# ross39/new_bloom_filter_repo

Hardware: AMD Instinct MI355X
Metric: Mpixels/s Bloom insert+query, 1080p residuals (higher is better)
Workload: dtype u64

## Files before the change

### new_bloom_filter_repo_amd/csrc/rbf_api.hip

```cpp
#include "rbf_host.h"
#include "rbf_kernels.h"
#include "rbf_kernels_noise.h"
#include "rbf_kernels_mask.h"
#include "rbf_kernels_hold.h"
#include "rbf_kernels_lookahead.h"
#include "rbf_kernels_barrett.h"
#include "rbf_kernels_insert_f64.h"
#include "rbf_kernels_reduce.h"
#include "rbf_kernels_query_f64.h"
#include "rbf_kernels_query_f64_tiled.h"
#include "rbf_kernels_witness.h"
#include "rbf_kernels_pack.h"
#include "rbf_kernels_digest.h"
#include "rbf_kernels_cut.h"
#include "rbf_rice_host.h"

#include <cmath>

struct MaskArgs {
    const void *frames; FrameLayout l; uint32_t nframes;
    int32_t thr_floor; const int32_t *thr_floors;
    void *masks; uint64_t mask_stride; uint64_t *ones;
    uint32_t channels;
};
// ... 103 lines not shown
    HIP_TRY(hipGetLastError());
    return RBF_OK;
}

static void launch_mask_gop(rbf_ctx *ctx, const MaskArgs &a, uint64_t fast_segs, uint32_t chunks, const MaskChunks &mc,
                            const int32_t *thr_tab_fast, const MaskFinish &fin)
{
    const uint32_t bx = (uint32_t)((fast_segs + WG_WAVES - 1) / WG_WAVES), pixel = a.l.pixel_stride;
    const size_t lds = (size_t)(a.nframes - 1) * 4;
    uint64_t *const acc = ctx->ones_acc.p;
    LaunchTimer t(ctx, RBF_K_MASK);
#define RBF_MASK_GOP(S, PB, Z) hipLaunchKernelGGL((k_residual_mask_gop<S, PB, true, Z>), dim3(bx, chunks), dim3(WG_THREADS), lds, ctx->stream,   \
                               (const uint8_t *)a.frames, a.l.frame_stride, a.nframes, fast_segs, a.thr_floor, thr_tab_fast,                    \
                               (uint16_t *)a.masks, a.mask_stride / 2, acc, mc, fin)
#define RBF_MASK_GOP2(S, PB) do { if (thr0) RBF_MASK_GOP(S, PB, true); else RBF_MASK_GOP(S, PB, false); } while (0)
#define RBF_MASK_ANY_GOP(S, PB) hipLaunchKernelGGL((k_residual_mask_any_gop<S, PB, true>), dim3(bx, chunks), dim3(WG_THREADS), lds, ctx->stream, \
                                (const uint8_t *)a.frames, a.l.frame_stride, a.nframes, fast_segs, thr_tab_fast, (uint16_t *)a.masks,           \
                                a.mask_stride / 2, acc, mc, fin)
    const bool thr0 = !thr_tab_fast && a.thr_floor == 0 && !ctx->knobs.force_generic_mask_bits;
    if (a.channels >= 2) {
        if (pixel == 3) RBF_MASK_ANY_GOP(uint8_t, 3);
        else if (pixel == 4) RBF_MASK_ANY_GOP(uint8_t, 4);
        else if (pixel == 6) RBF_MASK_ANY_GOP(uint16_t, 6);
        else RBF_MASK_ANY_GOP(uint16_t, 8);
    }
    else if (a.l.sample_bytes == 1 && pixel == 1) RBF_MASK_GOP2(uint8_t, 1);
    else if (a.l.sample_bytes == 1) RBF_MASK_GOP2(uint8_t, 3);
    else if (pixel == 2) RBF_MASK_GOP2(uint16_t, 2);
    else RBF_MASK_GOP2(uint16_t, 6);
#undef RBF_MASK_ANY_GOP
#undef RBF_MASK_GOP2
#undef RBF_MASK_GOP
}

static void launch_mask_generic(rbf_ctx *ctx, const MaskArgs &a, uint64_t first_word, const int32_t *thr_tab)
{
    const uint64_t n = (uint64_t)a.l.width * a.l.height, rest = (n + 63) / 64 - first_word;
    uint64_t bx = (rest + WG_WAVES * 16 - 1) / (WG_WAVES * 16);
    if (bx < 1) bx = 1;
    if (bx > 65535) bx = 65535;
    const dim3 grid((uint32_t)bx, a.nframes - 1), block(WG_THREADS);
    LaunchTimer t(ctx, RBF_K_MASK);
    by_sample_width(a.l.sample_bytes, [&](auto s) {
        using S = decltype(s);
        if (a.channels >= 2)
            hipLaunchKernelGGL(k_residual_mask_any<S>, grid, block, 0, ctx->stream, (const uint8_t *)a.frames, a.l.frame_stride, a.l.width, n,
                               a.l.row_pitch, a.l.pixel_stride, a.channels, thr_tab, (uint64_t *)a.masks, a.mask_stride / 8, ctx->ones_acc.p, first_word);
        else
            hipLaunchKernelGGL(k_residual_mask<S>, grid, block, 0, ctx->stream, (const uint8_t *)a.frames, a.l.frame_stride, a.l.width, n,
                               a.l.row_pitch, a.l.pixel_stride, a.thr_floor, thr_tab, (uint64_t *)a.masks, a.mask_stride / 8, ctx->ones_acc.p, first_word);
    });
}

static int prepare_mask_tickets(rbf_ctx *ctx)
{
    if (ctx->mask_ticket.p) return RBF_OK;
    if (int r = ctx->mask_ticket.alloc((MASK_TICKETS + 1) * 4)) return r;
    if (hipError_t e = hipMemsetAsync(ctx->mask_ticket.p, 0, (MASK_TICKETS + 1) * 4, ctx->stream)) {
        ctx->mask_ticket.release();
        return fail(RBF_EIO, "hipMemsetAsync(mask tickets): %s", hipGetErrorString(e));
    }
    return RBF_OK;
}

static int residual_mask_impl(rbf_ctx *ctx, const MaskArgs &a, bool finish, const MaskFinish *gop_tail = nullptr, const uint8_t *skip = nullptr)
{
    if (int r = set_device(ctx)) return r;
    if (int r = check_mask_args(a)) return r;
    const FrameLayout &l = a.l;
    const bool any = a.channels >= 2;
    const uint64_t n = (uint64_t)l.width * l.height, nwords = (n + 63) / 64;
    const uint32_t pairs = a.nframes - 1;
    if (int r = prepare_ones_acc(ctx, pairs)) return r;
    const bool flat = l.row_pitch == (uint64_t)l.width * l.pixel_stride;
    const bool known = any ? (a.channels * l.sample_bytes == l.pixel_stride && (a.channels == 3 || a.channels == 4))
                           : (l.sample_bytes == 1 && (l.pixel_stride == 1 || l.pixel_stride == 3)) ||
                             (l.sample_bytes == 2 && (l.pixel_stride == 2 || l.pixel_stride == 6));
    const bool fast = !ctx->knobs.force_generic && flat && known && l.frame_stride % 16 == 0 && ((uintptr_t)a.frames % 16) == 0 &&
                      (size_t)pairs * 4 <= 48 * 1024;
    const uint64_t fast_segs = fast ? n / 1024 : 0, first_word = fast_segs * 16;
    MaskChunks mc{};
    bool skip_in_table = false;
    const uint32_t chunks = fast_segs ? plan_mask_chunks(ctx->knobs, a.nframes, fast_segs, skip, &mc, &skip_in_table) : 1;
    const int32_t *thr_tab = nullptr, *thr_tab_fast = nullptr;
    if (a.thr_floors || (skip && (first_word < nwords || !skip_in_table))) {
        if (int r = store_thresholds(ctx, a, skip)) return r;
        thr_tab = ctx->thr_tab.p;
        if (a.thr_floors || (skip && !skip_in_table)) thr_tab_fast = ctx->thr_tab.p;
    }
    bool fused = false;
    if (fast_segs) {
        MaskFinish fin{};
        if (gop_tail && !ctx->knobs.no_fused_finish && first_word == nwords && !(((uintptr_t)gop_tail->clear_a | (uintptr_t)gop_tail->clear_b) & 15)) {
            if (int r = prepare_mask_tickets(ctx)) return r;
            fin = *gop_tail;
            fin.enabled = 1; fin.count = pairs; fin.ticket = ctx->mask_ticket.p; fin.ones_out = a.ones;
            fused = true;
        }
        launch_mask_gop(ctx, a, fast_segs, chunks, mc, thr_tab_fast, fin);
    }
    if (first_word < nwords) launch_mask_generic(ctx, a, first_word, thr_tab);
    HIP_TRY(hipGetLastError());
    if (fused) { ctx->ones_acc_dirty = false; return RBF_OK; }
    if (gop_tail) return launch_finish_ones(ctx, a.ones, pairs, gop_tail->host_block, gop_tail->token, gop_tail->clear_a, (size_t)gop_tail->quads_a * 16,
                                            gop_tail->clear_b, (size_t)gop_tail->quads_b * 16);
    if (finish) return launch_finish_ones(ctx, a.ones, pairs, nullptr, 0, nullptr, 0, nullptr, 0);
    return RBF_OK;
}

static int check_filter_strides(const rbf_filter_params *params, uint32_t nframes, uint64_t filter_stride_bytes)
{
    if (filter_stride_bytes % 8) return fail(RBF_EINVAL, "filter stride must be a multiple of 8");
    for (uint32_t f = 0; f < nframes; ++f) {
        const uint64_t need = (((uint64_t)params[f].m + 63) / 64) * 8;
        if (filter_stride_bytes < need)
            return fail(RBF_EINVAL, "frame %u: filter stride %llu < %llu", f, (unsigned long long)filter_stride_bytes, (unsigned long long)need);
    }
    return RBF_OK;
}

static int reserve_query_outputs(rbf_ctx *ctx, const Plan &pl, uint32_t nframes)
{
    if (WG_THREADS % pl.words_per_seg) return fail(RBF_EINVAL, "segments of %u words do not tile a workgroup's chunk", pl.words_per_seg);
    if (int r = ctx->pass_words.reserve((size_t)nframes * pl.nseg * pl.words_per_seg * 8)) return r;
    return ctx->seg_cnt.reserve((size_t)nframes * pl.nseg * 4 + 16);
}

static int launch_chunk_offsets(rbf_ctx *ctx, const Plan &pl, uint32_t nframes, uint32_t *nchunks,
                                void *witnesses_dev = nullptr , uint64_t witness_stride_bytes = 0)
{
    const uint64_t bx = std::max<uint64_t>(1, (pl.nseg * pl.words_per_seg + WG_THREADS - 1) / WG_THREADS);
    *nchunks = (uint32_t)bx;
    if (int r = ctx->chunk_off.reserve((size_t)nframes * bx * 4)) return r;
    LaunchTimer t(ctx, RBF_K_SCAN);
    hipLaunchKernelGGL(k_chunk_offsets, dim3(nframes), dim3(CO_THREADS), 0, ctx->stream, (const uint32_t *)ctx->seg_cnt.p, pl.nseg,
                       (uint32_t)WG_THREADS / pl.words_per_seg, *nchunks, ctx->chunk_off.p, (uint32_t *)witnesses_dev, witness_stride_bytes / 4);
    return RBF_OK;
}

struct QueryFlags {
    bool image_ready = false;
    bool table_for_next = false;
    bool quiet_passthrough = false;
};

static uint4 *table_to_rewrite(rbf_ctx *ctx, uint64_t n, const Seeds &sd)
{
    const SharedHashTable *sh = ctx->hash_shared;
    if (!sh || sh->n != n || !same_seeds(sh->seeds, sd) || ctx->knobs.no_hash_table || ctx->knobs.no_table_rewrite) return nullptr;
    std::lock_guard<std::mutex> lk(g_hash_mu);
    return sh->refs == 1 ? ctx->hash_tab : nullptr;
}

static int launch_query(rbf_ctx *ctx, const Plan &pl, const BloomBatch &b, const FrameTable &tab, const QueryFlags &flags)
{
    const uint32_t nframes = b.nframes;
    const Seeds sd = to_dev(*b.seeds);
    const uint32_t *filters = (const uint32_t *)b.filters;
    uint64_t stride_words = b.filter_stride / 4;
    if (pl.reads_probe_image()) {
        if (int r = ctx->qimage.reserve((size_t)nframes * pl.image_stride_words * 4)) return r;
        if (!flags.image_ready) {
            const uint32_t bx = (pl.image_stride_words + WG_THREADS - 1) / WG_THREADS;
            hipLaunchKernelGGL(k_probe_image, dim3(bx, nframes), dim3(WG_THREADS), 0, ctx->stream, filters, stride_words, ctx->qimage.p,
                               (uint64_t)pl.image_stride_words);
        }
        filters = ctx->qimage.p;
        stride_words = pl.image_stride_words;
    }
    const uint32_t lds_waves = (uint32_t)((pl.nseg + QL_WAVES - 1) / QL_WAVES);
    uint32_t nactive; uint64_t empty[2];
    LaunchTimer t(ctx, RBF_K_QUERY);
    if (pl.query == QueryKind::LdsTiledF64) {
        const FrameTable stab = query_table(tab, nframes, nullptr, &nactive, empty);
        if (flags.quiet_passthrough) empty[0] = empty[1] = 0;
        int mode = 0;
        for (uint32_t f = 0; f < nframes; ++f) {
            if (!tab.f[f].m) continue;
            if (tab.f[f].floor_k > 2) mode = 2;
            else if (tab.f[f].floor_k == 0 && mode < 1) mode = 1;
        }
        auto qkern = mode == 2 ? k_query_s64t<2> : mode == 1 ? k_query_s64t<1> : k_query_s64t<0>;
        if (int r = allow_big_lds((const void *)qkern)) return r;
        hipLaunchKernelGGL(qkern, dim3(lds_waves), dim3(QL_THREADS), s64t_lds_bytes(pl.query_tile_words), ctx->stream, b.n, nactive, stab, sd,
                           filters, stride_words, pl.query_tile_words, ctx->seg_cnt.p, pl.nseg, ctx->pass_words.p, empty[0], empty[1]);
    } else if (pl.reads_probe_image()) {
        uint4 *table_out = flags.table_for_next ? table_to_rewrite(ctx, b.n, sd) : nullptr;
        U64Classes cls;
        const FrameTable utab = query_table(tab, nframes, &cls, &nactive, empty);
        if (flags.quiet_passthrough) empty[0] = empty[1] = 0;
        const bool wide = cls.n[3] + cls.n[4] > 0;
        auto kern64 = wide ? k_query_u64w : k_query_u64;
        if (int r = allow_big_lds((const void *)kern64)) return r;
        hipLaunchKernelGGL(kern64, dim3(lds_waves), dim3(QL_THREADS), pl.query_lds_bytes + u64_geo_bytes(nactive), ctx->stream, b.n, nactive,
                           utab, cls, sd, filters, stride_words, pl.fwords_max, ctx->seg_cnt.p, pl.nseg, ctx->pass_words.p, table_out, empty[0],
                           empty[1]);
    } else if (pl.query == QueryKind::LdsWhole) {
        auto kern = pl.double_buffer ? (pl.small_m ? k_query_lds<true, true> : k_query_lds<true, false>)
                                     : (pl.small_m ? k_query_lds<false, true> : k_query_lds<false, false>);
        if (int r = allow_big_lds((const void *)kern)) return r;
        hipLaunchKernelGGL(kern, dim3(lds_waves), dim3(QL_THREADS), pl.query_lds_bytes, ctx->stream, b.n, nframes, tab, sd, filters, stride_words,
                           pl.fwords_max, ctx->seg_cnt.p, pl.nseg, ctx->pass_words.p);
    } else if (pl.query == QueryKind::LdsTiled) {
        auto kern = pl.small_m ? k_query_tiled<true> : k_query_tiled<false>;
        if (int r = allow_big_lds((const void *)kern)) return r;
        hipLaunchKernelGGL(kern, dim3(lds_waves), dim3(QL_THREADS), pl.query_lds_bytes, ctx->stream, b.n, nframes, tab, sd, filters, stride_words,
                           pl.query_tile_words, ctx->seg_cnt.p, pl.nseg, ctx->pass_words.p);
    } else {
        const uint64_t bx = (pl.nseg + WG_WAVES - 1) / WG_WAVES;
        hipLaunchKernelGGL(k_query, dim3((uint32_t)bx, nframes), dim3(WG_THREADS), 0, ctx->stream, b.n, tab, sd, filters, stride_words,
                           ctx->seg_cnt.p, pl.nseg, ctx->pass_words.p);
    }
    return RBF_OK;
}

static int launch_insert_positions(rbf_ctx *ctx, const BloomBatch &b, const FrameTable &itab, const Seeds &sd, bool hashed_positions)
{
    HIP_TRY(hipMemsetAsync(ctx->ins_counters.p, 0, (size_t)b.nframes * 4, ctx->stream));
    const uint64_t groups = (((b.n + 7) >> 3) + IT_STEP_BYTES - 1) / IT_STEP_BYTES;
    uint64_t S1 = (uint64_t)ctx->cus * 4 / (b.nframes ? b.nframes : 1);
    if (S1 > groups / (IP_WAVES * 4)) S1 = groups / (IP_WAVES * 4);
    S1 &= ~7ull;
    if (S1 < 1) S1 = 1;
    if (int r = allow_big_lds((const void *)k_insert_records)) return r;
    LaunchTimer t(ctx, RBF_K_INSERT);
    auto pkern = hashed_positions ? k_insert_positions<true> : k_insert_positions<false>;
    hipLaunchKernelGGL(pkern, dim3((uint32_t)S1, b.nframes), dim3(IP_THREADS), 0, ctx->stream, (const uint8_t *)b.masks, b.mask_stride, b.n, itab,
                       hashed_positions ? nullptr : (const uint4 *)ctx->hash_tab, sd, ctx->ins_records.p, ctx->ins_counters.p);
    return RBF_OK;
}

static bool settle_hash_table(rbf_ctx *ctx, const Plan &pl, const BloomBatch &b, const Seeds &sd)
{
    const bool table_too_big = hash_table_bytes(b.n) > HASH_TABLE_CACHE_BYTES;
    if (table_too_big || (pl.insert_two_phase && ctx->knobs.hash_positions)) {
        if (ctx->hash_shared && (ctx->hash_shared->n != b.n || !same_seeds(ctx->hash_shared->seeds, *b.seeds))) hash_table_release(ctx);
        return true;
    }
    bool built = false;
    if (!hash_table_acquire(ctx, b.n, *b.seeds, &built)) return true;
    if (ctx->knobs.hash_rebuild && !built) launch_hash_table(ctx, b.n, sd, ctx->hash_tab);
    return false;
}

static int insert_fast(rbf_ctx *ctx, const Plan &pl, const BloomBatch &b, const FrameTable &tab, const uint64_t *ones_host, bool stream_once,
                       uint32_t *image)
{
    const uint32_t nframes = b.nframes;
    const Seeds sd = to_dev(*b.seeds);
    const uint64_t part_stride = round_up4(pl.fwords_max);
    if (int r = ctx->partials.reserve((size_t)nframes * pl.S * part_stride * 4)) return r;
    const bool use_tab = pl.insert_tab;
    const bool hashed_positions = use_tab && settle_hash_table(ctx, pl, b, sd);
    const uint4 *hash_tab = hashed_positions ? nullptr : ctx->hash_tab;
    FrameTable itab = tab;
    if (use_tab)
        for (uint32_t f = 0; f < nframes; ++f)
            if (itab.f[f].m) { const double ninv = -1.0 / (double)itab.f[f].m; memcpy(&itab.f[f].M, &ninv, 8); }
    auto ikern = pl.small_m ? k_insert_lds<true> : k_insert_lds<false>;
    if (int r = allow_big_lds((const void *)ikern)) return r;
    const bool whole = pl.insert_tiles == 1;
    auto tkern = hashed_positions ? (whole ? k_insert_tab<true, true> : k_insert_tab<true, false>)
                                  : (whole ? k_insert_tab<false, true> : k_insert_tab<false, false>);
    if (int r = allow_big_lds((const void *)tkern)) return r;
    const bool two_phase = pl.insert_two_phase && use_tab;
    FrameTable rtab = tab;
    if (two_phase) {
        uint64_t first = 0;
        for (uint32_t f = 0; f < nframes; ++f) {
            itab.f[f].floor_k = (uint32_t)first;
            rtab.f[f].T = first;
            if (b.params[f].m) first += ones_host[f];
        }
        if (int r = launch_insert_positions(ctx, b, itab, sd, hashed_positions)) return r;
    }
    for (uint32_t f0 = 0; f0 < nframes;) {
        SliceTable grp{};
        uint32_t per_tile = 0, coded = 0, f = f0;
        for (; f < nframes && coded < pl.insert_group; ++f) {
            grp.n[f] = pl.slices.n[f];
            per_tile += grp.n[f];
            coded += grp.n[f] ? 1u : 0u;
        }
        f0 = f;
        if (!per_tile) continue;
        const dim3 grid(per_tile * pl.insert_tiles), block(IL_THREADS);
        LaunchTimer t(ctx, RBF_K_INSERT);
        if (two_phase)
            hipLaunchKernelGGL(k_insert_records, grid, block, pl.insert_lds_bytes, ctx->stream, (const uint2 *)ctx->ins_records.p,
                               (const uint32_t *)ctx->ins_counters.p, rtab, ctx->partials.p, part_stride, pl.insert_tile_words, grp, per_tile, pl.S);
        else if (use_tab)
            hipLaunchKernelGGL(tkern, grid, block, pl.insert_lds_bytes, ctx->stream, (const uint8_t *)b.masks, b.mask_stride, b.n, itab, hash_tab, sd,
                               ctx->partials.p, part_stride, pl.insert_tile_words, grp, per_tile, pl.S);
        else
            hipLaunchKernelGGL(ikern, grid, block, pl.insert_lds_bytes, ctx->stream, (const uint8_t *)b.masks, b.mask_stride, b.n, tab, sd,
                               ctx->partials.p, part_stride, pl.insert_tile_words, grp, per_tile, pl.S);
    }
    LaunchTimer t(ctx, RBF_K_REDUCE);
    const uint64_t words = b.filter_stride / 4;
    const uint32_t vec_ok = (words % 4 == 0 && ((uintptr_t)b.filters % 16) == 0) ? 1u : 0u;
    const uint32_t bx = std::max(1u, (uint32_t)((words + WG_THREADS * 4 - 1) / (WG_THREADS * 4)));
    hipLaunchKernelGGL(stream_once ? k_filter_reduce<true> : k_filter_reduce<false>, dim3(bx, nframes), dim3(WG_THREADS), 0, ctx->stream,
                       (const uint32_t *)ctx->partials.p, part_stride, pl.S, pl.slices, tab, (uint32_t *)b.filters, words, b.stats, vec_ok, image,
                       (uint64_t)pl.image_stride_words);
    return RBF_OK;
}

static int insert_generic(rbf_ctx *ctx, const Plan &pl, const BloomBatch &b, const FrameTable &tab, uint32_t *image)
{
    HIP_TRY(hipMemsetAsync(b.filters, 0, (size_t)b.nframes * b.filter_stride, ctx->stream));
    const uint64_t words = b.filter_stride / 4;
    const uint64_t bx = std::min<uint64_t>(((b.n + 31) / 32 + WG_THREADS - 1) / WG_THREADS, 65535);
    {
        LaunchTimer t(ctx, RBF_K_INSERT);
        hipLaunchKernelGGL(k_insert, dim3((uint32_t)bx, b.nframes), dim3(WG_THREADS), 0, ctx->stream, (const uint32_t *)b.masks, b.mask_stride / 4,
                           b.n, tab, to_dev(*b.seeds), (uint32_t *)b.filters, words);
    }
    LaunchTimer t(ctx, RBF_K_REDUCE);
    SliceTable ones;
    memset(ones.n, 1, sizeof ones.n);
    const uint32_t bx2 = std::max(1u, (uint32_t)((words + WG_THREADS * 4 - 1) / (WG_THREADS * 4)));
    hipLaunchKernelGGL(k_filter_reduce<false>, dim3(bx2, b.nframes), dim3(WG_THREADS), 0, ctx->stream, (const uint32_t *)b.filters, words, 1u, ones,
                       tab, (uint32_t *)b.filters, words, b.stats, 0u, image, (uint64_t)pl.image_stride_words);
    return RBF_OK;
}

static int encode_chunk_pass(rbf_ctx *ctx, const BloomBatch &b, bool outputs_zeroed, const uint64_t *ones_host, bool quiet_passthrough, bool compact)
{
    const uint32_t nframes = b.nframes;
    uint64_t nrecords = 0;
    uint32_t coded = 0;
    for (uint32_t f = 0; f < nframes; ++f) {
        if (!b.params[f].m) continue;
        ++coded;
        if (ones_host) nrecords += ones_host[f];
    }
    Plan pl = make_plan(ctx->knobs, ctx->cus, b.params, nframes, b.n, ones_host && nrecords < (1ull << 32));
    if (pl.insert_two_phase &&
        (ctx->ins_records.reserve((size_t)(nrecords ? nrecords : 1) * 8) || ctx->ins_counters.reserve((size_t)MAX_BATCH * 4))) {
        (void)hipGetLastError();
        pl = make_plan(ctx->knobs, ctx->cus, b.params, nframes, b.n, false);
    }
    FrameTable tab;
    if (int r = fill_table(b.params, nframes, &tab)) return r;
    const bool stream_once = (uint64_t)coded * b.n >= STREAM_MIN_PIXEL_FRAMES;
    if (int r = reserve_query_outputs(ctx, pl, nframes)) return r;
    if (int r = ctx->seg_off.reserve((size_t)nframes * pl.nseg * 8)) return r;
    const bool want_image = pl.reads_probe_image();
    if (want_image) if (int r = ctx->qimage.reserve((size_t)nframes * pl.image_stride_words * 4)) return r;
// ... 1110 lines not shown
```

### new_bloom_filter_repo_amd/csrc/rbf_kernels_query_f64.h

```cpp
#pragma once
#include "rbf_f64_common.h"
#include "rbf_kernels.h"
#include "rbf_lds_dma.h"
#include "rbf_query_f64_pass.h"

#include <type_traits>

namespace rbf {

template <bool ON>
struct RowDmaC {
    const uint8_t *image;
    uint32_t src;
    uint32_t dst_m0;
    uint64_t mask[5];
    bool full;

    __device__ __forceinline__ void issue() const
    {
        uint32_t keep; uint64_t keepx;
        if (full) {
            asm volatile("s_mov_b32 %0, m0\n\t"
                         "s_mov_b32 m0, %1\n\t"
                         "s_nop 0\n\t"
                         "global_load_lds_dwordx4 %2, %3 offset:-2048\n\t"
                         "global_load_lds_dwordx4 %2, %3 offset:-1024\n\t"
                         "global_load_lds_dwordx4 %2, %3\n\t"
                         "global_load_lds_dwordx4 %2, %3 offset:1024\n\t"
                         "global_load_lds_dwordx4 %2, %3 offset:2048\n\t"
                         "s_mov_b32 m0, %0"
                         : "=&s"(keep) : "s"(dst_m0), "v"(src), "s"(image) : "memory");
            return;
        }
        asm volatile("s_mov_b32 %0, m0\n\t"
                     "s_mov_b64 %1, exec\n\t"
                     "s_mov_b32 m0, %2\n\t"
                     "s_mov_b64 exec, %5\n\t"
                     "global_load_lds_dwordx4 %3, %4 offset:-2048\n\t"
                     "s_mov_b64 exec, %6\n\t"
                     "global_load_lds_dwordx4 %3, %4 offset:-1024\n\t"
                     "s_mov_b64 exec, %7\n\t"
                     "global_load_lds_dwordx4 %3, %4\n\t"
                     "s_mov_b64 exec, %8\n\t"
                     "global_load_lds_dwordx4 %3, %4 offset:1024\n\t"
                     "s_mov_b64 exec, %9\n\t"
                     "global_load_lds_dwordx4 %3, %4 offset:2048\n\t"
                     "s_mov_b64 exec, %1\n\t"
                     "s_mov_b32 m0, %0"
                     : "=&s"(keep), "=&s"(keepx)
                     : "s"(dst_m0), "v"(src), "s"(image), "s"(mask[0]), "s"(mask[1]), "s"(mask[2]), "s"(mask[3]), "s"(mask[4])
                     : "memory");
    }
    __device__ __forceinline__ void at(int g)
    {
        if (ON && g == 0) issue();
    }
};


template <bool WIDE>
__device__ __forceinline__ void query_u64_body(
    uint64_t n, uint32_t nactive, const FrameTable &tab, const U64Classes &cls, Seeds seeds,
    const uint32_t *__restrict__ image, uint64_t image_stride_words32, uint32_t fwords_max,
    uint32_t *__restrict__ seg_cnt, uint64_t nseg, uint64_t *__restrict__ pass_words,
    uint4 *__restrict__ table_out, uint64_t empty_lo, uint64_t empty_hi)
{
    extern __shared__ __attribute__((aligned(16))) uint32_t lds[];
    const uint32_t bufwords = ((fwords_max + 3u) & ~3u) + 4u;
    const uint32_t safe_pos = ((fwords_max + 3u) & ~3u) << 5;
    const uint32_t lane = threadIdx.x & 63u, wave = __builtin_amdgcn_readfirstlane(threadIdx.x >> 6);
    const uint32_t seg = blockIdx.x * QL_WAVES + wave;
    const bool live = seg < nseg;
    if (threadIdx.x < 8u) lds[(threadIdx.x >> 2) * bufwords + (bufwords - 4u) + (threadIdx.x & 3u)] = 0u;
    uint4 *geo = reinterpret_cast<uint4 *>(lds + 2u * bufwords);
    uint64_t *tl = reinterpret_cast<uint64_t *>(lds + bufwords);
    FrameDev fd_mine{};
    if (threadIdx.x < 2u * MAX_BATCH) fd_mine = tab.f[threadIdx.x < nactive ? threadIdx.x : 0u];

    static_assert(QL_P == 8, "a lane's verdicts fill one byte");
    double hd1[QL_P], hd2[QL_P];
    uint32_t hl1[QL_P], hl2[QL_P];
    uint32_t rank_lo = 0, rank_hi = 0;
    uint32_t validmask = 0;
    const uint64_t i0 = (uint64_t)seg * QL_SEG_PIXELS + (uint64_t)lane * QL_P;
    {
        uint64_t h1[QL_P], h2[QL_P], ha[QL_P];
#pragma unroll
        for (int it = 0; it < QL_P; ++it) {
            h1[it] = 0; h2[it] = 0; ha[it] = ~0ull;
            if (live && i0 + it < n) validmask |= 1u << it;
        }
        if (!hash3_run8((uint32_t)i0, validmask, seeds, h1, h2, ha)) {
#pragma unroll
            for (int it = 0; it < QL_P; ++it) {
                const bool act = (validmask >> it) & 1u;
                const Hash3 h = hash3_index((uint32_t)(i0 + it), act, seeds);
                h1[it] = h.h1; h2[it] = h.h2; ha[it] = h.ha;
            }
        }
#pragma unroll
        for (int it = 0; it < QL_P; ++it) {
            hd1[it] = (double)h1[it]; hl1[it] = (uint32_t)h1[it];
            hd2[it] = (double)h2[it]; hl2[it] = (uint32_t)h2[it];
        }
        if (table_out && live) hash_table_store8(table_out, n, seg, lane, h1, h2, ha);
        if (threadIdx.x < 2u * MAX_BATCH) {
            const uint32_t t = threadIdx.x;
            tl[t] = t < nactive ? fd_mine.T : ~0ull;
            if (t < nactive) {
                const uint32_t f = fd_mine.floor_k >> 16;
                const uint32_t row = (uint32_t)((uint64_t)f * image_stride_words32 * 4u);
                const uint32_t out_row = (uint32_t)((uint64_t)f * nseg);
                geo[2u * t] = make_uint4(fd_mine.m, (fd_mine.floor_k >> 8) & 0xFFu, (uint32_t)fd_mine.M, (uint32_t)(fd_mine.M >> 32));
                uint32_t *w = reinterpret_cast<uint32_t *>(geo);
                if (t) w[8u * (t - 1u) + 4u] = row;
                if (t + 1u == nactive) w[8u * t + 4u] = row;
                if (t == 0u) w[8u * nactive + 4u] = row;
                w[8u * t + 6u] = fd_mine.floor_k & 0xFFu;
                w[8u * (t + 1u) + 7u] = out_row;
            }
        }
        __syncthreads();
        uint32_t top = 1;
        while (2u * top <= nactive) top *= 2u;
        top = __builtin_amdgcn_readfirstlane(top);
        uint32_t r[QL_P];
#pragma unroll
        for (int it = 0; it < QL_P; ++it) r[it] = 0;
        for (uint32_t step = top; step; step >>= 1) {
#pragma unroll
            for (int it = 0; it < QL_P; ++it) {
                const uint64_t t = tl[r[it] + step - 1u];
                r[it] |= t <= ha[it] ? step : 0u;
            }
        }
        rank_lo = r[0] | (r[1] << 8) | (r[2] << 16) | (r[3] << 24);
        rank_hi = r[4] | (r[5] << 8) | (r[6] << 16) | (r[7] << 24);
    }
    const bool whole_wave = __builtin_amdgcn_readfirstlane((uint32_t)__all(validmask == 0xFFu)) != 0u;
    uint8_t *pass_bytes = reinterpret_cast<uint8_t *>(pass_words);

    for (uint32_t half = 0; half < 2; ++half) {
        uint64_t bits = half ? empty_hi : empty_lo;
        while (bits) {
            const uint32_t g = half * 64u + (uint32_t)__builtin_ctzll(bits);
            bits &= bits - 1;
            if (live && lane == 0) seg_cnt[(uint64_t)g * nseg + seg] = 0;
            if (live) pass_bytes[((uint64_t)g * nseg + seg) * (QL_SEG_PIXELS / 8) + lane] = 0;
        }
    }
    if (nactive == 0) return;

    const uint32_t lds0 = __builtin_amdgcn_readfirstlane(lds_addr_of(lds));
    const uint32_t pitch_bytes = (uint32_t)image_stride_words32 * 4u;
    const uint32_t off0 = wave * 5120u + lane * 16u;
    RowDmaC<true> dm;
    dm.image = reinterpret_cast<const uint8_t *>(image);
#pragma unroll
    for (int i = 0; i < 5; ++i) dm.mask[i] = __ballot(off0 + (uint32_t)i * 1024u + 16u <= pitch_bytes);
    dm.full = dm.mask[4] == ~0ull;
    const uint32_t off0b = off0 + 2048u, wave_dst = wave * 5120u + 2048u;
    const uint32_t buf_sum = lds0 + lds0 + bufwords * 4u;
    uint32_t fbase = vgpr_copy(lds0);
    {
        const uint32_t *w = reinterpret_cast<const uint32_t *>(geo);
        dm.src = w[8u * nactive + 4u] + off0 + 2048u;
        dm.dst_m0 = lds0 + wave * 5120u + 2048u;
        dm.at(0);
    }
    const uint32_t safe_v = vgpr_copy(safe_pos);
    const uint32_t seg_lane = seg * (QL_SEG_PIXELS / 8) + lane;
    uint32_t cnt2 = 0;
    uint32_t row_prev = 0, row_prev2 = 0;
    uint32_t out_row = 0;
    uint32_t out_pb = 0;
    bool out_pending = false, have_two = false;

    auto flush = [&]() {
        if (!out_pending) return;
        if (live) pass_bytes[(out_row << 6) + seg_lane] = (uint8_t)out_pb;
        {
            cnt2 = __builtin_amdgcn_alignbit(__popc(out_pb), cnt2, 16);
            row_prev2 = row_prev; row_prev = out_row;
            if (have_two) {
                const uint32_t tot = wave_sum_to_lane63(cnt2);
                if (live && lane == 63u) {
                    seg_cnt[row_prev2 + seg] = tot & 0xFFFFu;
                    seg_cnt[row_prev + seg] = tot >> 16;
                }
            }
            have_two = !have_two;
        }
    };

    uint32_t j = 0;
    auto frames = [&](auto fk_tag, uint32_t count) {
        constexpr int FK = decltype(fk_tag)::value;
        const uint32_t end = j + count;
        for (; j < end; ++j) {
            const uint4 ga = geo[2u * j], gb = geo[2u * j + 1u];
            const uint32_t m_v = ga.x, c_v = ga.y;
            const double ninv = __builtin_bit_cast(double, ((uint64_t)(uint32_t)__builtin_amdgcn_readfirstlane(ga.w) << 32) | (uint32_t)__builtin_amdgcn_readfirstlane(ga.z));
            uint32_t x[4] = {0, 0, 0, 0};
            const bool rows = FK > 0 && whole_wave;
            if (rows) rows_reduce4(0, hd1, hl1, hd2, hl2, m_v, ninv, x);
            dm.src = gb.x + off0b;
            dm.dst_m0 = (uint32_t)__builtin_amdgcn_readfirstlane(buf_sum - fbase) + wave_dst;
            dma_wait_all();
            out_row = (uint32_t)__builtin_amdgcn_readfirstlane(gb.w);
            __syncthreads();
            uint32_t pbf = 0;
            if (rows) {
                if constexpr (FK > 0) frame_pass_rows<FK, (FK < 5), true>(hd1, hl1, hd2, hl2, rank_lo, rank_hi, c_v, fbase, safe_v, m_v, ninv, x, pbf, dm, flush);
            } else {
                flush();
                const uint32_t fk = FK > 0 ? (uint32_t)FK : (uint32_t)__builtin_amdgcn_readfirstlane(gb.z);
                frame_pass_plain(hd1, hl1, hd2, hl2, rank_lo, rank_hi, c_v, validmask, fbase, safe_v, m_v, ninv, fk, pbf, dm);
            }
            out_pb = ~pbf & 0xFFu; out_pending = true;
            fbase = buf_sum - fbase;
        }
    };
    frames(std::integral_constant<int, 1>{}, cls.n[0]);
    frames(std::integral_constant<int, 2>{}, cls.n[1]);
    frames(std::integral_constant<int, 3>{}, cls.n[2]);
    if constexpr (WIDE) {
        frames(std::integral_constant<int, 4>{}, cls.n[3]);
        frames(std::integral_constant<int, 5>{}, cls.n[4]);
    }
    frames(std::integral_constant<int, 0>{}, cls.n[5] + (WIDE ? 0u : cls.n[3] + cls.n[4]));
    out_row = (uint32_t)__builtin_amdgcn_readfirstlane(reinterpret_cast<const uint32_t *>(geo)[8u * nactive + 7u]);
    flush();
    if (have_two) {
        const uint32_t tot = wave_sum_to_lane63(cnt2);
        if (live && lane == 63u) seg_cnt[row_prev + seg] = tot >> 16;
    }
}

#define RBF_U64_PARAMS uint64_t n, uint32_t nactive, const FrameTable tab, const U64Classes cls, Seeds seeds, const uint32_t *__restrict__ image, uint64_t image_stride_words32, \
    uint32_t fwords_max, uint32_t *__restrict__ seg_cnt, uint64_t nseg, uint64_t *__restrict__ pass_words, uint4 *__restrict__ table_out, uint64_t empty_lo, uint64_t empty_hi
#define RBF_U64_ARGS n, nactive, tab, cls, seeds, image, image_stride_words32, fwords_max, seg_cnt, nseg, pass_words, table_out, empty_lo, empty_hi
__attribute__((amdgpu_num_vgpr(60))) __global__ __launch_bounds__(QL_THREADS) void k_query_u64(RBF_U64_PARAMS) { query_u64_body<false>(RBF_U64_ARGS); }
__global__ __launch_bounds__(QL_THREADS) void k_query_u64w(RBF_U64_PARAMS) { query_u64_body<true>(RBF_U64_ARGS); }
#undef RBF_U64_PARAMS
#undef RBF_U64_ARGS

}
```

### new_bloom_filter_repo_amd/csrc/rbf_plan.h

```cpp
#pragma once
#include "../../include/rbf.h"
#include "rbf_geometry.h"

#include <algorithm>
#include <cstring>

using namespace rbf;

static int fail(int code, const char *fmt, ...);

struct Knobs {
    bool force_generic = false;
    bool single_buffer = false;
    bool force_generic_mask_bits = false;
    bool barrett_only = false;
    bool hash_rebuild = false;
    bool no_hash_table = false;
    bool no_two_phase = false;
    bool hash_positions = false;
    bool no_table_rewrite = false;
    bool no_fused_finish = false;
    uint32_t mask_chunks = 0;
    uint32_t tile_words = 0;
    uint32_t insert_slices = 0;
    void set_flags(int on)
    {
        force_generic = on & 1;
        single_buffer = on & 2;
        force_generic_mask_bits = on & 4;
        barrett_only = on & 8;
        hash_rebuild = on & 16;
        no_hash_table = on & 32;
        no_two_phase = on & 128;
        mask_chunks = (uint32_t)(on >> 8) & 0x1F;
        hash_positions = on & (1 << 14);
        no_table_rewrite = on & (1 << 15);
        tile_words = ((uint32_t)on >> 16) << 6;
    }
    bool fp64_kernels() const { return !force_generic && !barrett_only && !single_buffer; }
};

static inline FrameDev frame_dev(const rbf_filter_params &p)
{
    return FrameDev{p.m, p.floor_k, p.threshold, p.m >= 2 ? (uint64_t)((((unsigned __int128)1) << 64) / p.m) : 0};
}

static int fill_table(const rbf_filter_params *params, uint32_t count, FrameTable *tab)
{
    memset(tab, 0, sizeof *tab);
    for (uint32_t f = 0; f < count; ++f) {
        if (params[f].floor_k > 64) return fail(RBF_ERANGE, "frame %u: floor_k %u > 64", f, params[f].floor_k);
        tab->f[f] = frame_dev(params[f]);
    }
    return RBF_OK;
}

static FrameTable query_table(const FrameTable &tab, uint32_t nframes, U64Classes *cls, uint32_t *nactive, uint64_t (&empty)[2])
{
    FrameTable q;
    memset(&q, 0, sizeof q);
    if (cls) memset(cls, 0, sizeof *cls);
    empty[0] = empty[1] = 0;
    uint64_t sorted[MAX_BATCH];
    uint32_t coded = 0;
    for (uint32_t f = 0; f < nframes; ++f) {
        if (tab.f[f].m) sorted[coded++] = tab.f[f].T;
        else empty[f >> 6] |= 1ull << (f & 63);
    }
    std::sort(sorted, sorted + coded);
    uint32_t j = 0;
    for (int k = 0; k < (cls ? U64_CLASSES : 1); ++k)
        for (uint32_t f = 0; f < nframes; ++f) {
            if (!tab.f[f].m) continue;
            const uint32_t fk = tab.f[f].floor_k;
            if (cls && (fk >= 1u && fk <= 5u ? (int)fk - 1 : 5) != k) continue;
            const double ninv = -1.0 / (double)tab.f[f].m;
            const uint32_t below = (uint32_t)(std::lower_bound(sorted, sorted + coded, tab.f[f].T) - sorted);
            q.f[j].m = tab.f[f].m;
            memcpy(&q.f[j].M, &ninv, 8);
            q.f[j].floor_k = (fk & 0xFFu) | (below << 8) | (f << 16);
            q.f[j].T = sorted[j];
            if (cls) ++cls->n[k];
            ++j;
        }
    *nactive = coded;
    return q;
}

constexpr size_t LDS_LIMIT = 160 * 1024;
constexpr size_t HASH_TABLE_CACHE_BYTES = (size_t)96 << 20;
constexpr uint32_t MAX_INSERT_TILES = 7, MAX_QUERY_TILES = 3;
constexpr uint64_t STREAM_MIN_PIXEL_FRAMES = 64ull * 1920 * 1080;

enum class QueryKind {
    Generic,
    LdsWhole,
    LdsTiled,
    LdsTiledF64,
};

struct Plan {
    bool fast_insert;
    QueryKind query;
    bool double_buffer, small_m;
    bool insert_tab;
    bool insert_two_phase;
    bool f64_mod;
    uint32_t fwords_max, S , per_tile , insert_group ;
    SliceTable slices;
    uint32_t insert_tile_words, insert_tiles, query_tile_words;
    size_t insert_lds_bytes, query_lds_bytes;
    uint64_t nseg; uint32_t words_per_seg;
    uint32_t image_stride_words;
    bool reads_probe_image() const { return (query == QueryKind::LdsWhole || query == QueryKind::LdsTiledF64) && f64_mod; }
};

static inline uint32_t round_up4(uint32_t words) { return (words + 3u) & ~3u; }
static inline bool in_f64_range(uint32_t m) { return m >= F64MOD_M_MIN && m <= F64MOD_M_MAX; }
static inline size_t hash_table_bytes(uint64_t n) { return ((size_t)n + QL_SEG_PIXELS) * 32; }

static uint32_t tile_words_for(uint32_t fwords, uint32_t cap, uint32_t knob, bool even)
{
    uint32_t tw = round_up4(fwords);
    if (tw > cap) {
        const uint32_t nt = (fwords + cap - 1) / cap;
        tw = even ? round_up4((fwords + nt - 1) / nt) : cap;
    }
    if (knob && knob < tw) tw = knob & ~3u;
    return tw < 4 ? 4 : tw;
}

struct BatchSizes {
    uint32_t mmax = 0, active = 0;
    bool small_m = true;
    bool all_f64 = true;
};

static BatchSizes classify(const rbf_filter_params *params, uint32_t nframes)
{
    BatchSizes b;
    for (uint32_t f = 0; f < nframes; ++f) {
        const uint32_t m = params[f].m;
        if (m > b.mmax) b.mmax = m;
        if (m) ++b.active;
        if (m == 1 || m > (1u << 30)) b.small_m = false;
        if (m && !in_f64_range(m)) b.all_f64 = false;
    }
    return b;
}

static void plan_insert_tiles(Plan &p, const Knobs &k, const BatchSizes &b, bool have_ones)
{
    const size_t queue_bytes = (size_t)IL_WAVES * (IT_WAVE_LDS_BYTES > IL_QUEUE * 4 ? IT_WAVE_LDS_BYTES : IL_QUEUE * 4);
    p.insert_tile_words = tile_words_for(p.fwords_max, (uint32_t)((LDS_LIMIT - queue_bytes) / 4) & ~3u, k.tile_words, false);
    p.insert_lds_bytes = (size_t)p.insert_tile_words * 4 + queue_bytes;
    p.insert_tiles = std::max(1u, (p.fwords_max + p.insert_tile_words - 1) / p.insert_tile_words);
    p.fast_insert = !k.force_generic && b.mmax > 0 && !(k.tile_words == 0 && p.insert_tiles > MAX_INSERT_TILES);
    p.insert_tab = p.fast_insert && b.all_f64 && !k.no_hash_table && !k.barrett_only;
    p.insert_two_phase = p.insert_tab && !k.no_two_phase && have_ones && p.insert_tiles > 1;
    if (p.insert_two_phase) {
        p.insert_tile_words = tile_words_for(p.fwords_max, (uint32_t)(LDS_LIMIT / 4) & ~3u, k.tile_words, true);
        p.insert_tiles = (p.fwords_max + p.insert_tile_words - 1) / p.insert_tile_words;
        p.insert_lds_bytes = (size_t)p.insert_tile_words * 4;
    }
}

static void plan_query(Plan &p, const Knobs &k, const BatchSizes &b, uint32_t nframes, uint64_t n)
{
    const size_t fbytes = (size_t)round_up4(p.fwords_max) * 4;
    const bool lds = !k.force_generic && b.mmax > 0;
    const bool u64_offsets_fit = (uint64_t)nframes * ((n + QL_SEG_PIXELS - 1) / QL_SEG_PIXELS) * (QL_SEG_PIXELS / 8) < (1ull << 32);
    p.f64_mod = b.all_f64 && !k.barrett_only && !k.single_buffer && u64_offsets_fit &&
                2 * (fbytes + 16) + u64_geo_bytes(nframes) <= LDS_LIMIT;
    const size_t qbytes = fbytes + (p.f64_mod ? 16 : 0);
    p.double_buffer = 2 * qbytes <= LDS_LIMIT && !k.single_buffer;
    p.query = QueryKind::Generic;
    if (lds && qbytes <= LDS_LIMIT && !k.tile_words) {
        p.query = QueryKind::LdsWhole;
        p.query_lds_bytes = (p.double_buffer ? 2 : 1) * qbytes;
    } else if (lds) {
        p.query = QueryKind::LdsTiled;
        p.query_tile_words = (uint32_t)(LDS_LIMIT / 4);
        if (k.tile_words && k.tile_words < p.query_tile_words) p.query_tile_words = k.tile_words & ~3u;
        if (p.query_tile_words < 4) p.query_tile_words = 4;
        p.query_lds_bytes = (size_t)std::min(p.query_tile_words, round_up4(p.fwords_max)) * 4;
        if (k.tile_words == 0 && (p.fwords_max + p.query_tile_words - 1) / p.query_tile_words > MAX_QUERY_TILES) p.query = QueryKind::Generic;
    }
// ... 62 lines not shown
```

Baseline: 557,800.

## Read precomputed hash table in u64 query instead of recomputing hashes

Adds table-reading variants of the u64 probe-image query kernel. They load precomputed hash positions and 16-bit tags from the shared hash table instead of running hash3 per pixel. Frame ranking uses a 16-bit tag binary search, falling back to the full 64-bit activation search only on ties. The first row DMA is issued before the table loads to overlap them. This trades hash arithmetic for extra global reads of the table, and relies on the table matching the current seeds and n.

After: 570,200 (median of 6 runs). 1.02x the previous value.

```diff
diff --git a/new_bloom_filter_repo_amd/csrc/rbf_api.hip b/new_bloom_filter_repo_amd/csrc/rbf_api.hip
--- a/new_bloom_filter_repo_amd/csrc/rbf_api.hip
+++ b/new_bloom_filter_repo_amd/csrc/rbf_api.hip
@@ -279,6 +279,13 @@
     return sh->refs == 1 ? ctx->hash_tab : nullptr;
 }
 
+static const uint4 *table_for_query(rbf_ctx *ctx, const BloomBatch &b)
+{
+    const SharedHashTable *sh = ctx->hash_shared;
+    if (!sh || !sh->is_for(ctx->device, b.n, *b.seeds) || ctx->knobs.no_hash_table || ctx->knobs.query_hashes) return nullptr;
+    return ctx->hash_tab;
+}
+
 static int launch_query(rbf_ctx *ctx, const Plan &pl, const BloomBatch &b, const FrameTable &tab, const QueryFlags &flags)
 {
     const uint32_t nframes = b.nframes;
@@ -312,16 +319,25 @@
         hipLaunchKernelGGL(qkern, dim3(lds_waves), dim3(QL_THREADS), s64t_lds_bytes(pl.query_tile_words), ctx->stream, b.n, nactive, stab, sd,
                            filters, stride_words, pl.query_tile_words, ctx->seg_cnt.p, pl.nseg, ctx->pass_words.p, empty[0], empty[1]);
     } else if (pl.reads_probe_image()) {
-        uint4 *table_out = flags.table_for_next ? table_to_rewrite(ctx, b.n, sd) : nullptr;
+        const uint4 *table_in = table_for_query(ctx, b);
+        uint4 *table_out = flags.table_for_next && !table_in ? table_to_rewrite(ctx, b.n, sd) : nullptr;
         U64Classes cls;
         const FrameTable utab = query_table(tab, nframes, &cls, &nactive, empty);
         if (flags.quiet_passthrough) empty[0] = empty[1] = 0;
         const bool wide = cls.n[3] + cls.n[4] > 0;
-        auto kern64 = wide ? k_query_u64w : k_query_u64;
-        if (int r = allow_big_lds((const void *)kern64)) return r;
-        hipLaunchKernelGGL(kern64, dim3(lds_waves), dim3(QL_THREADS), pl.query_lds_bytes + u64_geo_bytes(nactive), ctx->stream, b.n, nactive,
-                           utab, cls, sd, filters, stride_words, pl.fwords_max, ctx->seg_cnt.p, pl.nseg, ctx->pass_words.p, table_out, empty[0],
-                           empty[1]);
+        if (table_in) {
+            auto kern64 = wide ? k_query_u64w_tab : k_query_u64_tab;
+            if (int r = allow_big_lds((const void *)kern64)) return r;
+            hipLaunchKernelGGL(kern64, dim3(lds_waves), dim3(QL_THREADS), pl.query_lds_bytes + u64_geo_bytes(nactive), ctx->stream, b.n, nactive,
+                               utab, cls, sd, filters, stride_words, pl.fwords_max, ctx->seg_cnt.p, pl.nseg, ctx->pass_words.p, table_in,
+                               ctx->knobs.query_all_ties ? 1u : 0u, empty[0], empty[1]);
+        } else {
+            auto kern64 = wide ? k_query_u64w : k_query_u64;
+            if (int r = allow_big_lds((const void *)kern64)) return r;
+            hipLaunchKernelGGL(kern64, dim3(lds_waves), dim3(QL_THREADS), pl.query_lds_bytes + u64_geo_bytes(nactive), ctx->stream, b.n, nactive,
+                               utab, cls, sd, filters, stride_words, pl.fwords_max, ctx->seg_cnt.p, pl.nseg, ctx->pass_words.p, table_out, empty[0],
+                               empty[1]);
+        }
     } else if (pl.query == QueryKind::LdsWhole) {
         auto kern = pl.double_buffer ? (pl.small_m ? k_query_lds<true, true> : k_query_lds<true, false>)
                                      : (pl.small_m ? k_query_lds<false, true> : k_query_lds<false, false>);
diff --git a/new_bloom_filter_repo_amd/csrc/rbf_kernels_query_f64.h b/new_bloom_filter_repo_amd/csrc/rbf_kernels_query_f64.h
--- a/new_bloom_filter_repo_amd/csrc/rbf_kernels_query_f64.h
+++ b/new_bloom_filter_repo_amd/csrc/rbf_kernels_query_f64.h
@@ -58,12 +58,12 @@
 };
 
 
-template <bool WIDE>
+template <bool WIDE, bool TAB>
 __device__ __forceinline__ void query_u64_body(
     uint64_t n, uint32_t nactive, const FrameTable &tab, const U64Classes &cls, Seeds seeds,
     const uint32_t *__restrict__ image, uint64_t image_stride_words32, uint32_t fwords_max,
     uint32_t *__restrict__ seg_cnt, uint64_t nseg, uint64_t *__restrict__ pass_words,
-    uint4 *__restrict__ table_out, uint64_t empty_lo, uint64_t empty_hi)
+    uint4 *__restrict__ table_out, const uint4 *__restrict__ table_in, uint32_t all_ties, uint64_t empty_lo, uint64_t empty_hi)
 {
     extern __shared__ __attribute__((aligned(16))) uint32_t lds[];
     const uint32_t bufwords = ((fwords_max + 3u) & ~3u) + 4u;
@@ -76,6 +76,48 @@
     uint64_t *tl = reinterpret_cast<uint64_t *>(lds + bufwords);
     FrameDev fd_mine{};
     if (threadIdx.x < 2u * MAX_BATCH) fd_mine = tab.f[threadIdx.x < nactive ? threadIdx.x : 0u];
+    uint8_t *pass_bytes = reinterpret_cast<uint8_t *>(pass_words);
+    auto write_empties = [&]() {
+        for (uint32_t half = 0; half < 2; ++half) {
+            uint64_t bits = half ? empty_hi : empty_lo;
+            while (bits) {
+                const uint32_t g = half * 64u + (uint32_t)__builtin_ctzll(bits);
+                bits &= bits - 1;
+                if (live && lane == 0) seg_cnt[(uint64_t)g * nseg + seg] = 0;
+                if (live) pass_bytes[((uint64_t)g * nseg + seg) * (QL_SEG_PIXELS / 8) + lane] = 0;
+            }
+        }
+    };
+
+    uint32_t lds0 = 0, off0b = 0, wave_dst = 0, buf_sum = 0, fbase = 0;
+    RowDmaC<true> dm;
+    auto stager_setup = [&]() {
+        lds0 = __builtin_amdgcn_readfirstlane(lds_addr_of(lds));
+        const uint32_t pitch_bytes = (uint32_t)image_stride_words32 * 4u;
+        const uint32_t off0 = wave * 5120u + lane * 16u;
+        dm.image = reinterpret_cast<const uint8_t *>(image);
+#pragma unroll
+        for (int i = 0; i < 5; ++i) dm.mask[i] = __ballot(off0 + (uint32_t)i * 1024u + 16u <= pitch_bytes);
+        dm.full = dm.mask[4] == ~0ull;
+        off0b = off0 + 2048u; wave_dst = wave * 5120u + 2048u;
+        buf_sum = lds0 + lds0 + bufwords * 4u;
+        fbase = vgpr_copy(lds0);
+    };
+
+    uint4 e[QL_P] = {};
+    uint4 tg = {};
+    const uint32_t seg_ld = live ? seg : 0u;
+    if constexpr (TAB) {
+        if (nactive == 0) { write_empties(); return; }
+        stager_setup();
+        dm.src = (uint32_t)((uint64_t)(tab.f[0].floor_k >> 16) * image_stride_words32 * 4u) + off0b;
+        dm.dst_m0 = lds0 + wave_dst;
+        dm.issue();
+        const HashTable t(const_cast<uint4 *>(table_in), n);
+        tg = reinterpret_cast<const uint4 *>(t.tag)[seg_ld * (QL_SEG_PIXELS / QL_P) + lane];
+#pragma unroll
+        for (int it = 0; it < QL_P; ++it) e[it] = t.pos[(uint64_t)seg_ld * QL_SEG_PIXELS + (uint32_t)it * 64u + lane];
+    }
 
     static_assert(QL_P == 8, "a lane's verdicts fill one byte");
     double hd1[QL_P], hd2[QL_P];
@@ -90,23 +132,30 @@
             h1[it] = 0; h2[it] = 0; ha[it] = ~0ull;
             if (live && i0 + it < n) validmask |= 1u << it;
         }
-        if (!hash3_run8((uint32_t)i0, validmask, seeds, h1, h2, ha)) {
+        if constexpr (!TAB) {
+            if (!hash3_run8((uint32_t)i0, validmask, seeds, h1, h2, ha)) {
+#pragma unroll
+                for (int it = 0; it < QL_P; ++it) {
+                    const bool act = (validmask >> it) & 1u;
+                    const Hash3 h = hash3_index((uint32_t)(i0 + it), act, seeds);
+                    h1[it] = h.h1; h2[it] = h.h2; ha[it] = h.ha;
+                }
+            }
 #pragma unroll
             for (int it = 0; it < QL_P; ++it) {
-                const bool act = (validmask >> it) & 1u;
-                const Hash3 h = hash3_index((uint32_t)(i0 + it), act, seeds);
-                h1[it] = h.h1; h2[it] = h.h2; ha[it] = h.ha;
-            }
-        }
-#pragma unroll
-        for (int it = 0; it < QL_P; ++it) {
-            hd1[it] = (double)h1[it]; hl1[it] = (uint32_t)h1[it];
-            hd2[it] = (double)h2[it]; hl2[it] = (uint32_t)h2[it];
-        }
-        if (table_out && live) hash_table_store8(table_out, n, seg, lane, h1, h2, ha);
+                hd1[it] = (double)h1[it]; hl1[it] = (uint32_t)h1[it];
+                hd2[it] = (double)h2[it]; hl2[it] = (uint32_t)h2[it];
+            }
+            if (table_out && live) hash_table_store8(table_out, n, seg, lane, h1, h2, ha);
+        }
+        uint32_t *tt = reinterpret_cast<uint32_t *>(tl + 2u * MAX_BATCH);
         if (threadIdx.x < 2u * MAX_BATCH) {
             const uint32_t t = threadIdx.x;
             tl[t] = t < nactive ? fd_mine.T : ~0ull;
+            if constexpr (TAB) {
+                tt[t + 1u] = t < nactive ? (uint32_t)(fd_mine.T >> 48) : 0x10000u;
+                if (t == 0u) tt[0] = 0x10000u;
+            }
             if (t < nactive) {
                 const uint32_t f = fd_mine.floor_k >> 16;
                 const uint32_t row = (uint32_t)((uint64_t)f * image_stride_words32 * 4u);
@@ -127,45 +176,53 @@
         uint32_t r[QL_P];
 #pragma unroll
         for (int it = 0; it < QL_P; ++it) r[it] = 0;
-        for (uint32_t step = top; step; step >>= 1) {
+        if constexpr (!TAB) {
+            for (uint32_t step = top; step; step >>= 1) {
+#pragma unroll
+                for (int it = 0; it < QL_P; ++it) {
+                    const uint64_t t = tl[r[it] + step - 1u];
+                    r[it] |= t <= ha[it] ? step : 0u;
+                }
+            }
+        } else {
+            const uint32_t tw[4] = {tg.x, tg.y, tg.z, tg.w};
+            uint32_t tag[QL_P];
+#pragma unroll
+            for (int it = 0; it < QL_P; ++it) tag[it] = (it & 1) ? tw[it >> 1] >> 16 : tw[it >> 1] & 0xFFFFu;
+            for (uint32_t step = top; step; step >>= 1) {
+#pragma unroll
+                for (int it = 0; it < QL_P; ++it) r[it] |= tt[r[it] + step] <= tag[it] ? step : 0u;
+            }
+            const HashTable t(const_cast<uint4 *>(table_in), n);
 #pragma unroll
             for (int it = 0; it < QL_P; ++it) {
-                const uint64_t t = tl[r[it] + step - 1u];
-                r[it] |= t <= ha[it] ? step : 0u;
+                const bool tie = tt[r[it]] == tag[it];
+                if (__any(tie) || all_ties) {
+                    const uint64_t h = t.act[(uint64_t)seg_ld * QL_SEG_PIXELS + (uint32_t)it * 64u + lane];
+                    uint32_t rr = 0;
+                    for (uint32_t step = top; step; step >>= 1) rr |= tl[rr + step - 1u] <= h ? step : 0u;
+                    r[it] = rr;
+                }
             }
         }
         rank_lo = r[0] | (r[1] << 8) | (r[2] << 16) | (r[3] << 24);
         rank_hi = r[4] | (r[5] << 8) | (r[6] << 16) | (r[7] << 24);
     }
     const bool whole_wave = __builtin_amdgcn_readfirstlane((uint32_t)__all(validmask == 0xFFu)) != 0u;
-    uint8_t *pass_bytes = reinterpret_cast<uint8_t *>(pass_words);
-
-    for (uint32_t half = 0; half < 2; ++half) {
-        uint64_t bits = half ? empty_hi : empty_lo;
-        while (bits) {
-            const uint32_t g = half * 64u + (uint32_t)__builtin_ctzll(bits);
-            bits &= bits - 1;
-            if (live && lane == 0) seg_cnt[(uint64_t)g * nseg + seg] = 0;
-            if (live) pass_bytes[((uint64_t)g * nseg + seg) * (QL_SEG_PIXELS / 8) + lane] = 0;
-        }
-    }
+
+    write_empties();
     if (nactive == 0) return;
-
-    const uint32_t lds0 = __builtin_amdgcn_readfirstlane(lds_addr_of(lds));
-    const uint32_t pitch_bytes = (uint32_t)image_stride_words32 * 4u;
-    const uint32_t off0 = wave * 5120u + lane * 16u;
-    RowDmaC<true> dm;
-    dm.image = reinterpret_cast<const uint8_t *>(image);
-#pragma unroll
-    for (int i = 0; i < 5; ++i) dm.mask[i] = __ballot(off0 + (uint32_t)i * 1024u + 16u <= pitch_bytes);
-    dm.full = dm.mask[4] == ~0ull;
-    const uint32_t off0b = off0 + 2048u, wave_dst = wave * 5120u + 2048u;
-    const uint32_t buf_sum = lds0 + lds0 + bufwords * 4u;
-    uint32_t fbase = vgpr_copy(lds0);
-    {
+    if constexpr (TAB) {
+#pragma unroll
+        for (int it = 0; it < QL_P; ++it) {
+            hd1[it] = rn_double(e[it].x, e[it].y); hl1[it] = e[it].x;
+            hd2[it] = rn_double(e[it].z, e[it].w); hl2[it] = e[it].z;
+        }
+    } else {
+        stager_setup();
         const uint32_t *w = reinterpret_cast<const uint32_t *>(geo);
-        dm.src = w[8u * nactive + 4u] + off0 + 2048u;
-        dm.dst_m0 = lds0 + wave * 5120u + 2048u;
+        dm.src = w[8u * nactive + 4u] + off0b;
+        dm.dst_m0 = lds0 + wave_dst;
         dm.at(0);
     }
     const uint32_t safe_v = vgpr_copy(safe_pos);
@@ -238,10 +295,24 @@
 }
 
 #define RBF_U64_PARAMS uint64_t n, uint32_t nactive, const FrameTable tab, const U64Classes cls, Seeds seeds, const uint32_t *__restrict__ image, uint64_t image_stride_words32, \
-    uint32_t fwords_max, uint32_t *__restrict__ seg_cnt, uint64_t nseg, uint64_t *__restrict__ pass_words, uint4 *__restrict__ table_out, uint64_t empty_lo, uint64_t empty_hi
-#define RBF_U64_ARGS n, nactive, tab, cls, seeds, image, image_stride_words32, fwords_max, seg_cnt, nseg, pass_words, table_out, empty_lo, empty_hi
-__attribute__((amdgpu_num_vgpr(60))) __global__ __launch_bounds__(QL_THREADS) void k_query_u64(RBF_U64_PARAMS) { query_u64_body<false>(RBF_U64_ARGS); }
-__global__ __launch_bounds__(QL_THREADS) void k_query_u64w(RBF_U64_PARAMS) { query_u64_body<true>(RBF_U64_ARGS); }
+    uint32_t fwords_max, uint32_t *__restrict__ seg_cnt, uint64_t nseg, uint64_t *__restrict__ pass_words
+#define RBF_U64_ARGS n, nactive, tab, cls, seeds, image, image_stride_words32, fwords_max, seg_cnt, nseg, pass_words
+__attribute__((amdgpu_num_vgpr(60))) __global__ __launch_bounds__(QL_THREADS) void k_query_u64(RBF_U64_PARAMS, uint4 *__restrict__ table_out, uint64_t empty_lo, uint64_t empty_hi)
+{
+    query_u64_body<false, false>(RBF_U64_ARGS, table_out, nullptr, 0u, empty_lo, empty_hi);
+}
+__global__ __launch_bounds__(QL_THREADS) void k_query_u64w(RBF_U64_PARAMS, uint4 *__restrict__ table_out, uint64_t empty_lo, uint64_t empty_hi)
+{
+    query_u64_body<true, false>(RBF_U64_ARGS, table_out, nullptr, 0u, empty_lo, empty_hi);
+}
+__attribute__((amdgpu_num_vgpr(60))) __global__ __launch_bounds__(QL_THREADS) void k_query_u64_tab(RBF_U64_PARAMS, const uint4 *__restrict__ table, uint32_t all_ties, uint64_t empty_lo, uint64_t empty_hi)
+{
+    query_u64_body<false, true>(RBF_U64_ARGS, nullptr, table, all_ties, empty_lo, empty_hi);
+}
+__global__ __launch_bounds__(QL_THREADS) void k_query_u64w_tab(RBF_U64_PARAMS, const uint4 *__restrict__ table, uint32_t all_ties, uint64_t empty_lo, uint64_t empty_hi)
+{
+    query_u64_body<true, true>(RBF_U64_ARGS, nullptr, table, all_ties, empty_lo, empty_hi);
+}
 #undef RBF_U64_PARAMS
 #undef RBF_U64_ARGS
 
diff --git a/new_bloom_filter_repo_amd/csrc/rbf_plan.h b/new_bloom_filter_repo_amd/csrc/rbf_plan.h
--- a/new_bloom_filter_repo_amd/csrc/rbf_plan.h
+++ b/new_bloom_filter_repo_amd/csrc/rbf_plan.h
@@ -19,6 +19,8 @@
     bool no_two_phase = false;
     bool hash_positions = false;
     bool no_table_rewrite = false;
+    bool query_hashes = false;
+    bool query_all_ties = false;
     bool no_fused_finish = false;
     uint32_t mask_chunks = 0;
     uint32_t tile_words = 0;
@@ -31,8 +33,10 @@
         barrett_only = on & 8;
         hash_rebuild = on & 16;
         no_hash_table = on & 32;
+        query_hashes = on & 64;
         no_two_phase = on & 128;
         mask_chunks = (uint32_t)(on >> 8) & 0x1F;
+        query_all_ties = on & (1 << 13);
         hash_positions = on & (1 << 14);
         no_table_rewrite = on & (1 << 15);
         tile_words = ((uint32_t)on >> 16) << 6;
```
